# yekaizhou/duet

Measured on AMD Instinct MI355X. Metric: SV support-read marks clustered+phased /sec; bit-exact phased_sv.vcf vs ref, higher is better.
Workload: dtype u32/u64 integer + f64 threshold compares; 1 GPU; BASELINE configs[1]: synthetic 1 contig, 1001116 SV marks / 100000 candidates / 159991 tagged reads, resident in HBM; step = ef_classify + ef_finalize_own, two launches (phasing, E/F; ef_seed_sort 0: ; marks_per_gpu=1001116, candidates_per_gpu=100000, reads_per_gpu=159991, parallelism=contig-sharded x1, svlen_thres=50, suppread_thres=2, device_preheat_steps=2700

## Files before the change

### duet_amd/csrc/duet_ef.hip

```cpp

#include <hip/hip_runtime.h>
#include <hip/hip_ext.h>
#include <stdint.h>
#include <stdio.h>
#include <stdlib.h>
#include <string.h>
#include <string>
#include <vector>

#include "duet_ef.h"
#include "duet_internal.h"

#pragma clang fp contract(off)

namespace {

#ifdef DUET_STAMPS
#define STAMP(k, i) do { if (threadIdx.x == 0 && p.stamps) p.stamps[((size_t)(k) * 65536 + blockIdx.x) * 8 + (i)] = wall_clock64(); } while (0)
#else
#define STAMP(k, i) do { } while (0)
#endif

#include "duet_seeds.hip.h"

// ... 295 lines not shown
    const uint32_t s_a1 = a1 ? wave_sum(ta1) : 0u, s_a2 = a2 ? wave_sum(ta2) : 0u;
    const uint32_t s_b1 = b1 ? wave_sum(tb1) : 0u, s_b2 = b2 ? wave_sum(tb2) : 0u;
    if (lane == h) {
        st.first_ps = first_ps; st.multi = st.multi || multi;
        st.ps_a = ps_a; st.ps_b = ps_b; st.more = st.more || more;
        st.nv += nv; st.n_a += n_a; st.n_b += n_b;
        st.a1 += a1; st.a2 += a2; st.b1 += b1; st.b2 += b2;
        st.TA1 += s_a1; st.TA2 += s_a2; st.tb1 += s_b1; st.tb2 += s_b2;
    }
}

__device__ __forceinline__ void lds_barrier() { asm volatile("s_waitcnt lgkmcnt(0)\n\ts_barrier" ::: "memory"); }

struct TileRecs {
    const ulonglong4 *p;
    __device__ __forceinline__ ulonglong4 operator[](uint32_t b) const { return p[2 * (size_t)b]; }
    __device__ __forceinline__ ulonglong4 second(uint32_t b) const { return p[2 * (size_t)b + 1]; }
};

struct TileShared {
    uint32_t seed[kCandPerBlock];
    uint32_t wcnt[kCandPerBlock / 64], wlast[kCandPerBlock / 64], wclean[kCandPerBlock / 64];
    uint32_t c2n;
    uint32_t c2base;
};

__device__ __forceinline__ void store_summary(const Params &p, uint32_t slot, const CandState &st)
{
    uint32_t *rec = p.c2rec + (size_t)slot * kC2Words;
    const uint32_t ng = (st.n_a != 0) + (st.n_b != 0);
    rec[0] = st.nv; rec[1] = ng;
    rec[2] = st.ps_a; rec[3] = st.n_a; rec[4] = st.a1; rec[5] = st.a2;
    rec[6] = (uint32_t)st.TA1; rec[7] = (uint32_t)st.TA2;
    rec[8] = st.ps_b; rec[9] = st.n_b; rec[10] = st.b1; rec[11] = st.b2; rec[12] = st.tb1; rec[13] = st.tb2;
}

__device__ __forceinline__ uint32_t decide_store(const Params &p, TileShared &sh, uint32_t tile, bool live, uint32_t c,
                                                 bool active, bool divzero, const CandState &st, uint32_t deg,
                                                 uint32_t svread, uint32_t refread, uint32_t &c2_rank)
{
    uint8_t code = 0;
    uint32_t ps_out = 0;
    bool want_seed = false;
    const uint32_t n_ps = st.n_ps();
    const bool c2 = active && n_ps == 2;
    const bool c2_fast = c2 && !st.more && deg < 500000u;
    const uint32_t rank = c2_fast ? atomicAdd(&sh.c2n, 1u) : kEmpty;
    c2_rank = rank;
    if (live) {
        want_seed = (active || divzero) && (n_ps == 1) && st.seed() != kEmpty;
        if (divzero) {
            code = kDivZero;
        } else if (active) {
            if (c2) {
                if (rank < kC2Quota) {
                    const uint32_t slot = tile * kC2Quota + rank;
                    store_summary(p, slot, st);
                    code = kClass2;
                    ps_out = slot;
                } else {
                    code = kClass2Slow;
                }
            } else {
                Vote v;
                v.hap1 = st.a1; v.hap2 = st.a2; v.hap0 = 0;
                v.allhap = st.a1 + st.a2;
                v.t1 = st.TA1; v.t2 = st.TA2;
                bool need_fp = false;
                int pred = (p.dbg & DUET_DBG_EF_FP_DECIDE) ? 0 : decide01_int((int)n_ps, v, deg, svread, refread, need_fp);
                need_fp = need_fp || (p.dbg & DUET_DBG_EF_FP_DECIDE) != 0;
                if (need_fp) pred = decide((int)n_ps, v, deg, svread, refread);
                code = (uint8_t)pred;
                ps_out = st.ps_a == kEmpty ? 0u : st.ps_a;
                if (n_ps == 0 || (st.a1 == 0 && st.a2 == 0)) code |= kNeedNearest;
            }
        }
        p.out_pred[c] = code;
        p.out_ps[c] = ps_out;
    }
    return want_seed ? st.seed() : kEmpty;
}

__device__ __forceinline__ void seeds_tile(const Params &p, TileShared &sh, uint32_t tile, uint32_t tid, uint32_t c,
                                           uint32_t is_start)
{
    const uint32_t seed = sh.seed[tid];
    const bool want_seed = seed != kEmpty;
    const uint32_t lane = tid & 63u, wave = tid >> 6;
    const unsigned long long wmask = __ballot(want_seed);
    const unsigned long long smask = __ballot(is_start != 0);
    const unsigned long long upto = lane == 63 ? ~0ull : ((1ull << (lane + 1)) - 1ull);
    if (lane == 0) {
        if (wmask) {
            const uint32_t li = 63u - (uint32_t)__clzll(wmask);
            sh.wlast[wave] = sh.seed[wave * 64 + li];
            sh.wclean[wave] = (li == 63 || (smask >> (li + 1)) == 0) ? 1u : 0u;
        } else {
            sh.wlast[wave] = kEmpty;
            sh.wclean[wave] = 0;
        }
    }
    __syncthreads();
    bool keep = want_seed;
    if (want_seed) {
        const unsigned long long lower = wmask & (upto >> 1);
        if (lower) {
            const uint32_t pl = 63u - (uint32_t)__clzll(lower);
            const unsigned long long between = smask & upto & ~((1ull << (pl + 1)) - 1ull);
            keep = !(between == 0 && sh.seed[wave * 64 + pl] == seed);
        } else if (wave > 0) {
            keep = !((smask & upto) == 0 && sh.wclean[wave - 1] && sh.wlast[wave - 1] == seed);
        }
    }
    const unsigned long long mask = __ballot(keep);
    if (lane == 0) sh.wcnt[wave] = (uint32_t)__popcll(mask);
    __syncthreads();
    uint32_t before = 0, total = 0;
#pragma unroll
    for (uint32_t w = 0; w < kCandPerBlock / 64; ++w) {
        before += w < wave ? sh.wcnt[w] : 0u;
        total += sh.wcnt[w];
    }
    if (keep) {
        const uint32_t at = before + (uint32_t)__popcll(mask & (upto >> 1));
        const uint64_t e = ((uint64_t)c << 32) | seed;
        if (at < 7) p.blk_rec[(size_t)tile * 8 + 1 + at] = e;
        if (at >= 3) p.seed_ent[(size_t)tile * kCandPerBlock + at] = e;
    }
    if (tid == 0) p.blk_rec[(size_t)tile * 8] = total;
}

__device__ __forceinline__ void issue_fence()
{
    asm volatile("" ::: "memory");
    __builtin_amdgcn_sched_barrier(0);
}

__device__ __forceinline__ void stage_load_marks(const uint32_t *__restrict__ mark_read, uint4 (&r)[kStageIt], uint32_t cs, uint32_t m_end,
                                                 uint32_t tid)
{
#pragma unroll
    for (int it = 0; it < kStageIt; ++it) {
        const uint32_t m = cs + 4u * (tid + it * kCandPerBlock);
        r[it] = *reinterpret_cast<const uint4 *>(mark_read + (m < m_end ? m : cs));
    }
    issue_fence();
}

__device__ __forceinline__ void stage_gather(const uint64_t *__restrict__ read_tag, const uint64_t *__restrict__ untagged, uint32_t n_reads,
                                             uint64_t (&t)[4 * kStageIt], const uint4 (&r)[kStageIt])
{
#pragma unroll
    for (int it = 0; it < kStageIt; ++it) {
        uint32_t idx[4] = {r[it].x, r[it].y, r[it].z, r[it].w};
        asm volatile("" : "+v"(idx[0]), "+v"(idx[1]), "+v"(idx[2]), "+v"(idx[3])::"memory");
#pragma unroll
        for (int j = 0; j < 4; ++j) {
            const uint64_t *a = idx[j] < n_reads ? read_tag + idx[j] : untagged;
            t[4 * it + j] = *a;
        }
        issue_fence();
    }
}

__device__ __forceinline__ void stage_store(uint64_t *s_tag, const uint64_t (&t)[4 * kStageIt], uint32_t tid)
{
#pragma unroll
    for (int it = 0; it < kStageIt; ++it) {
        const uint32_t i = 4u * (tid + it * kCandPerBlock);
#pragma unroll
        for (int j = 0; j < 4; ++j) s_tag[i + j] = t[4 * it + j];
    }
}

template <bool VEC, bool DYN = false>
__global__ __launch_bounds__(kCandPerBlock, 6) void ef_classify(const Params p)
{
    __shared__ uint64_t s_tag[kChunk];
    __shared__ uint32_t s_span[2];
    __shared__ TileShared sh;

    const uint32_t tid = threadIdx.x;
    STAMP(0, 0);
    const uint32_t C = p.C, n_reads = p.n_reads, svlen_thres = p.svlen_thres, suppread_thres = p.suppread_thres;
    const uint32_t heavy_t = min(p.heavy_t, 255u);
    const uint32_t *__restrict__ const cand_off = p.cand_off, *__restrict__ const mark_read = p.mark_read;
    const uint64_t *__restrict__ const read_tag = p.read_tag, *__restrict__ const untagged = p.untagged;
    const uint32_t *__restrict__ const cand_svlen = p.cand_svlen, *__restrict__ const cand_svread = p.cand_svread;
    const uint32_t *__restrict__ const cand_refread = p.cand_refread;
    const uint8_t *__restrict__ const cand_gt_ok = p.cand_gt_ok, *__restrict__ const ctg_start = p.ctg_start;
    asm volatile("" ::"s"(C), "s"(n_reads), "s"(svlen_thres), "s"(suppread_thres), "s"(heavy_t), "s"(cand_off), "s"(mark_read),
                 "s"(read_tag), "s"(untagged), "s"(cand_svlen), "s"(cand_svread), "s"(cand_refread), "s"(cand_gt_ok), "s"(ctg_start));
    asm volatile("" ::"s"(p.dbg), "s"(p.out_pred), "s"(p.out_ps), "s"(p.blk_rec), "s"(p.seed_ent), "s"(p.c2rec), "s"(p.status),
                 "s"(p.c2_fixed), "s"(p.c2_cap));
    uint32_t n_cands = C;
    for (uint32_t tile = blockIdx.x;; tile += gridDim.x) {
        const uint32_t c0 = tile * kCandPerBlock, c = c0 + tid;
        const uint32_t ic = min(c, C - 1u);
        const uint32_t o0_ld = cand_off[min(c, C)], o1_ld = cand_off[min(c + 1u, C)];
        const uint32_t svlen_ld = cand_svlen[ic], svread_ld = cand_svread[ic], refread_ld = cand_refread[ic], gt_ld = cand_gt_ok[ic];
        uint32_t start_ld = 0, cc0_ld = 0, cc1_ld = 0, mb_ld = 0, me_ld = 0;
        if constexpr (DYN) {
            if (p.cand_contig) {
                cc0_ld = p.cand_contig[ic];
                cc1_ld = p.cand_contig[max(ic, 1u) - 1u];
            }
        } else {
            start_ld = ctg_start[ic];
            mb_ld = cand_off[c0];
            me_ld = cand_off[min(c0 + (uint32_t)kCandPerBlock, C)];
        }
        if constexpr (DYN) {
            uint32_t zero = 0;
            asm volatile("" : "+s"(zero));
            n_cands = p.dyn_c[zero];
            if (c0 >= n_cands) break;
        }
        const uint32_t nc = min((uint32_t)kCandPerBlock, n_cands - c0);
        asm volatile("" ::"v"(o0_ld), "v"(o1_ld), "v"(svlen_ld), "v"(svread_ld), "v"(refread_ld), "v"(gt_ld), "v"(start_ld), "v"(cc0_ld),
                     "v"(cc1_ld));
        if (tid == 0) sh.c2n = 0;
        const bool live = tid < nc;
        const uint32_t svlen = svlen_ld, svread = svread_ld, refread = refread_ld, gt_ok = gt_ld;
        uint32_t is_start = 0;
        if constexpr (DYN) {
            if (p.cand_contig) {
                is_start = (live && (c == 0 || cc0_ld != cc1_ld)) ? 1u : 0u;
            } else if (live) {
                uint32_t k = p.blk_ctg[tile];
                while (c >= p.ctg_off[k + 1]) ++k;
                is_start = c == p.ctg_off[k] ? 1u : 0u;
            }
        } else {
            is_start = live ? start_ld : 0u;
        }
        const bool kept = live && svlen >= svlen_thres && svread >= suppread_thres && gt_ok != 0;
        const bool divzero = kept && ((uint64_t)svread + (uint64_t)refread == 0);
        uint32_t m_begin, m_end;
        if constexpr (DYN) {
            if (tid == 0) s_span[0] = o0_ld;
            if (tid == nc - 1u) s_span[1] = o1_ld;
            lds_barrier();
            m_begin = s_span[0]; m_end = s_span[1];
        } else {
            m_begin = mb_ld; m_end = me_ld;
        }
        m_begin = (uint32_t)__builtin_amdgcn_readfirstlane((int)m_begin);
        m_end = (uint32_t)__builtin_amdgcn_readfirstlane((int)m_end);
        STAMP(0, 1);

        const uint32_t j = tid;
        const bool active = kept && !divzero;
        const uint32_t my_b = live ? o0_ld : 0, my_e = live ? o1_ld : 0;
        CandState st;

        const uint32_t base = VEC ? (m_begin & ~3u) : m_begin;
        for (uint32_t cs = base; cs < m_end; cs += kChunk) {
            if (VEC) {
                uint4 r[kStageIt];
                uint64_t t[4 * kStageIt];
                stage_load_marks(mark_read, r, cs, m_end, tid);
                stage_gather(read_tag, untagged, n_reads, t, r);
                stage_store(s_tag, t, tid);
            } else {
                for (uint32_t i = tid; i < kChunk && cs + i < m_end; i += kCandPerBlock) {
                    const uint32_t r = mark_read[cs + i];
                    s_tag[i] = r < n_reads ? read_tag[r] : kUntagged;
                }
            }
            __syncthreads();
            STAMP(0, 2);
            uint32_t lo = max(my_b, cs);
            const uint32_t hi = min(my_e, cs + (uint32_t)kChunk);
            if (!kept) lo = hi;
            const bool heavy = lo < hi && my_e - my_b > heavy_t;
            unsigned long long hm = __ballot(heavy);
            consume_range(st, s_tag, heavy ? hi : lo, hi, cs);
            while (hm) {
                const uint32_t h = (uint32_t)__builtin_amdgcn_readfirstlane((int)((uint32_t)__ffsll((long long)hm) - 1u));
                hm &= hm - 1ull;
                const uint32_t lo_h = (uint32_t)__builtin_amdgcn_readlane((int)lo, h), hi_h = (uint32_t)__builtin_amdgcn_readlane((int)hi, h);
                consume_heavy(st, s_tag, lo_h, hi_h, cs, tid & 63u, h);
            }
            STAMP(0, 3);
            __syncthreads();
        }
        STAMP(0, 4);
        uint32_t c2_rank;
        const uint32_t seed = decide_store(p, sh, tile, live, c0 + j, active, divzero, st, my_e - my_b, svread, refread, c2_rank);
        sh.seed[j] = seed;
        __syncthreads();
        if (sh.c2n > kC2Quota) {
            if (tid == 0) sh.c2base = atomicAdd(&p.status[1], sh.c2n - kC2Quota);
            __syncthreads();
            if (live && c2_rank != kEmpty && c2_rank >= kC2Quota) {
                const uint32_t at = sh.c2base + (c2_rank - kC2Quota);
                if (at < p.c2_cap - p.c2_fixed) {
                    store_summary(p, p.c2_fixed + at, st);
                    p.out_pred[c0 + j] = kClass2;
                    p.out_ps[c0 + j] = p.c2_fixed + at;
                }
            }
        }
        seeds_tile(p, sh, tile, tid, c0 + tid, is_start);
        STAMP(0, 6);
        if (!DYN) break;
        __syncthreads();
    }
}


__device__ void bitonic_sort(uint32_t *a, uint32_t n, uint32_t tid, uint32_t nthreads)
{
    uint32_t lN = 0;
    while ((1u << lN) < n) ++lN;
    const uint32_t pairs = (1u << lN) >> 1;
    for (uint32_t lk = 1; lk <= lN; ++lk) {
        const uint32_t k = 1u << lk, half = k >> 1;
        for (uint32_t i = tid; i < pairs; i += nthreads) {
            const uint32_t base = (i >> (lk - 1)) << lk, off = i & (half - 1);
            const uint32_t x = base + off, y = base + (k - 1 - off);
            if (y < n) {
                const uint32_t ax = a[x], ay = a[y];
                if (ax > ay) { a[x] = ay; a[y] = ax; }
            }
        }
        __syncthreads();
        for (int lj = (int)lk - 2; lj >= 0; --lj) {
            const uint32_t j = 1u << lj;
            for (uint32_t i = tid; i < pairs; i += nthreads) {
                const uint32_t x = ((i >> lj) << (lj + 1)) + (i & (j - 1)), y = x + j;
                if (y < n) {
                    const uint32_t ax = a[x], ay = a[y];
                    if (ax > ay) { a[x] = ay; a[y] = ax; }
                }
            }
            __syncthreads();
        }
    }
}

__device__ bool oddeven_rounds(uint32_t *a, uint32_t n, uint32_t tid, uint32_t nthreads, uint32_t *s_flag, int max_rounds)
{
    for (int r = 0; r < max_rounds; ++r) {
        if (tid == 0) *s_flag = 0;
        __syncthreads();
        for (int par = 0; par < 2; ++par) {
            for (uint32_t i = 2 * tid + par; i + 1 < n; i += 2 * nthreads) {
                const uint32_t x = a[i], y = a[i + 1];
                if (x > y) { a[i] = y; a[i + 1] = x; *s_flag = 1; }
            }
            __syncthreads();
        }
        if (*s_flag == 0) return true;
        __syncthreads();
    }
    return false;
}

__device__ uint32_t block_exscan(uint32_t v, uint32_t tid, uint32_t *s_part , uint32_t nthreads,
                                 uint32_t *total)
{
    const uint32_t lane = tid & 63u, wave = tid >> 6;
    uint32_t x = v;
#pragma unroll
    for (int d = 1; d < 64; d <<= 1) {
        const uint32_t y = __shfl_up(x, d, 64);
        if ((int)lane >= d) x += y;
    }
    if (lane == 63) s_part[wave] = x;
    __syncthreads();
    uint32_t before = 0, tot = 0;
    for (uint32_t w = 0; w < nthreads / 64; ++w) {
        const uint32_t pw = s_part[w];
        before += w < wave ? pw : 0u;
        tot += pw;
    }
    __syncthreads();
    *total = tot;
    return before + x - v;
}

__device__ uint32_t unique_copy(const uint32_t *src, uint32_t n, uint32_t *dst, uint32_t tid, uint32_t nthreads,
                                uint32_t *s_part)
{
    const uint32_t per = (n + nthreads - 1) / nthreads;
    const uint32_t b = min(n, tid * per), e = min(n, b + per);
    uint32_t cnt = 0;
    for (uint32_t i = b; i < e; ++i) cnt += (i == 0 || src[i] != src[i - 1]);
    uint32_t total;
    uint32_t at = block_exscan(cnt, tid, s_part, nthreads, &total);
// ... 1349 lines not shown
    if (ctx->cl_fork) (void)hipEventDestroy(ctx->cl_fork);
    if (ctx->sv_depth_off_ev) (void)hipEventDestroy(ctx->sv_depth_off_ev);
    if (ctx->plan_ev) (void)hipEventDestroy(ctx->plan_ev);
    if (ctx->plan_stage) (void)hipHostFree(ctx->plan_stage);
    delete ctx;
}

int duet_ctx_set_profiling(duet_ctx *ctx, int enabled)
{
    if (!ctx) return fail(nullptr, DUET_ERR_INVALID, "null context");
    if (ctx->ev_used && ctx->ev_mode != (enabled == 3 ? 1 : enabled))
        return fail(ctx, DUET_ERR_INVALID, "collect the pending profile before changing the mode");
    ctx->profiling = enabled < 0 ? 0 : (enabled > 3 ? 3 : enabled);
    ctx->prof_tick = 0;
    return DUET_OK;
}

#ifdef DUET_STAMPS
DUET_API int duet_dbg_stamps(duet_ctx *ctx, int enable, unsigned long long *host_out)
{
    const size_t bytes = (size_t)6 * 65536 * 8 * 8;
    if (enable && !ctx->d_stamps) { if (hipMalloc((void **)&ctx->d_stamps, bytes) != hipSuccess) return -1; }
    if (enable) { (void)hipMemset(ctx->d_stamps, 0, bytes); return 0; }
    if (ctx->d_stamps && host_out) { (void)hipDeviceSynchronize(); (void)hipMemcpy(host_out, ctx->d_stamps, bytes, hipMemcpyDeviceToHost); }
    return 0;
}
#endif

int duet_ctx_set_debug(duet_ctx *ctx, uint32_t flags)
{
    if (!ctx) return fail(nullptr, DUET_ERR_INVALID, "null context");
    ctx->dbg = flags;
    return DUET_OK;
}

int duet_ef_run_device(duet_ctx *ctx, const duet_ef_problem *pr, uint8_t *out_pred, uint32_t *out_ps, void *stream_)
{
    int rc = validate(ctx, pr, out_pred, out_ps);
    if (rc) return rc;
    hipStream_t stream = (hipStream_t)stream_;
    HIP_TRY(ctx, hipSetDevice(ctx->device));
    if (pr->n_cands == 0) return DUET_OK;
    if ((rc = ensure_plan(ctx, pr, stream))) return rc;

    Params p;
    memset(&p, 0, sizeof(p));
    p.K = pr->n_contigs; p.C = pr->n_cands; p.M = pr->n_marks;
    p.read_tag = pr->n_reads ? pr->read_tag : (const uint64_t *)ctx->d_n_one;
    p.n_reads = pr->n_reads; p.untagged = ctx->d_untagged;
    p.cand_pos = pr->cand_pos; p.cand_svlen = pr->cand_svlen; p.cand_svread = pr->cand_svread;
    p.cand_refread = pr->cand_refread; p.cand_gt_ok = pr->cand_gt_ok;
    p.cand_off = pr->cand_off; p.mark_read = pr->mark_read;
    p.svlen_thres = pr->svlen_thres; p.suppread_thres = pr->suppread_thres;
    p.ctg_off = ctx->d_ctg_off; p.ctg_start = (const uint8_t *)ctx->ws_start.ptr; p.blk_ctg = ctx->d_blk_ctg;
    p.blk_rec = (uint64_t *)ctx->d_blk_cnt; p.seed_ent = (uint64_t *)ctx->ws_ent.ptr;
    p.one_cap = pr->n_cands + pr->n_contigs;
    p.n_small = pr->n_contigs <= (uint32_t)kSmallK ? pr->n_contigs : 0;
    for (uint32_t k = 0; k <= p.n_small && p.n_small; ++k) p.ctg_small[k] = pr->cand_ctg_off[k];
    p.onebuf = (uint32_t *)ctx->ws_one.ptr; p.tmpbuf = (uint32_t *)ctx->ws_tmp.ptr;
    p.n_one = ctx->d_n_one; p.c2rec = (uint32_t *)ctx->ws_c2.ptr; p.status = ctx->d_status;
    p.c2_fixed = ((p.C + kCandPerBlock - 1) / kCandPerBlock) * kC2Quota;
    p.c2_cap = (uint32_t)c2_slots((p.C + kCandPerBlock - 1) / kCandPerBlock, p.C);
    p.out_pred = out_pred; p.out_ps = out_ps;
    p.dbg = ctx->dbg;
    p.heavy_t = (ctx->dbg & DUET_DBG_EF_HEAVY_ALL) ? 0u : ((ctx->dbg & DUET_DBG_EF_HEAVY_OFF) ? 0xFFFFFFFFu : ctx->ef_heavy_t);
    p.stamps = ctx->d_stamps;

    hipEvent_t ev[6] = {nullptr, nullptr, nullptr, nullptr, nullptr, nullptr};
    int prof = ctx->profiling;
    if (prof == 3) prof = (ctx->prof_tick++ % 8u == 0) ? 1 : 0;
    if (prof) {
        ctx->ev_mode = prof;
        while (ctx->ev_pool.size() < ctx->ev_used + 6) {
            hipEvent_t e;
            HIP_TRY(ctx, hipEventCreate(&e));
            ctx->ev_pool.push_back(e);
        }
        for (int i = 0; i < (prof == 2 ? 6 : 2); ++i) ev[i] = ctx->ev_pool[ctx->ev_used + i];
        ctx->ev_used += 6;
    }
    const uint32_t blocks = (pr->n_cands + kCandPerBlock - 1) / kCandPerBlock;
    const uint32_t three = DUET_DBG_EF_OWN_OFF | DUET_DBG_EF_FIN_TPB2 | DUET_DBG_EF_FIN_TPB4 | DUET_DBG_EF_NO_SEED_HASH;
    const bool own = p.n_small && !(ctx->dbg & three) && (blocks <= kOwnMaxTiles || (ctx->dbg & DUET_DBG_EF_OWN_ALL));
    if (prof) ctx->ev_kmask.push_back(own ? 0x5 : 0x7);
    if (((uintptr_t)pr->mark_read & 15) == 0)
        hipExtLaunchKernelGGL(ef_classify<true>, dim3(blocks), dim3(kCandPerBlock), 0, stream, ev[0], ev[1], 0, p);
    else
        hipExtLaunchKernelGGL(ef_classify<false>, dim3(blocks), dim3(kCandPerBlock), 0, stream, ev[0], ev[1], 0, p);
    if (own) {
        hipExtLaunchKernelGGL(ef_finalize_own, dim3(blocks), dim3(256), 0, stream, ev[4], ev[5], 0, p);
        ctx->ef_last_params.assign((const unsigned char *)&p, (const unsigned char *)&p + sizeof(p));
        ctx->ef_last_stream = stream;
        ctx->ef_seeds_stale = true;
    } else {
        ctx->ef_seeds_stale = false;
        hipExtLaunchKernelGGL(ef_seed_sort, dim3(pr->n_contigs), dim3(kSortThreads), 0, stream, ev[2], ev[3], 0, p);
        const uint32_t C = pr->n_cands;
        int tpb = (!p.n_small || C < 1000000u) ? 1 : (C < 8000000u ? 2 : 4);
        if (p.n_small && (ctx->dbg & DUET_DBG_EF_FIN_TPB2)) tpb = 2;
        if (p.n_small && (ctx->dbg & DUET_DBG_EF_FIN_TPB4)) tpb = 4;
        if (tpb == 4) hipExtLaunchKernelGGL((ef_finalize<false, 4>), dim3((C + 1023) / 1024), dim3(256), 0, stream, ev[4], ev[5], 0, p);
        else if (tpb == 2) hipExtLaunchKernelGGL((ef_finalize<false, 2>), dim3((C + 511) / 512), dim3(256), 0, stream, ev[4], ev[5], 0, p);
        else hipExtLaunchKernelGGL((ef_finalize<false, 1>), dim3((C + 255) / 256), dim3(256), 0, stream, ev[4], ev[5], 0, p);
    }
    HIP_TRY(ctx, hipGetLastError());
    ctx->pending_check = true;
    return DUET_OK;
}

}

int duet_ef_plan_on_device_prepare(duet_ctx *ctx, uint32_t K, uint32_t c_max, hipStream_t stream, uint32_t **ctg_off_out,
                                   uint32_t **zero_out)
{
    const uint32_t C = c_max;
    const uint32_t B = (C + kCandPerBlock - 1) / kCandPerBlock;
    const size_t small_words = (size_t)(K + 1) + K + 8 + (size_t)B + 16 + (size_t)B * 16;
    const size_t want[6] = {small_words * 4, C, (size_t)B * kCandPerBlock * 8, ((size_t)C + K + 1) * 4, ((size_t)C + K + 1) * 4,
                            c2_slots(B, C) * kC2Words * 4};
    DevBuf *bufs[6] = {&ctx->ws_small, &ctx->ws_start, &ctx->ws_ent, &ctx->ws_one, &ctx->ws_tmp, &ctx->ws_c2};
    bool grow = ctx->plan_stream != stream;
    for (int i = 0; i < 6; ++i) grow = grow || want[i] > bufs[i]->cap;
    int rc;
    if (grow) {
        HIP_TRY(ctx, hipDeviceSynchronize());
        for (int i = 0; i < 6; ++i)
            if ((rc = reserve(ctx, *bufs[i], want[i]))) return rc;
    }
    uint32_t *w = (uint32_t *)ctx->ws_small.ptr;
    ctx->d_ctg_off = w;            w += K + 1;
    ctx->d_n_one = w;              w += K;
    ctx->d_status = w;             w += 8;
    ctx->d_blk_ctg = w;            w += B;
    w += ((uintptr_t)w & 63) ? (64 - ((uintptr_t)w & 63)) / 4 : 0;
    ctx->d_blk_cnt = w;
    ctx->plan_off.clear();
    ctx->plan_C = 0;
    ctx->plan_stream = stream;
    if (ctg_off_out) *ctg_off_out = ctx->d_ctg_off;
    if (zero_out) *zero_out = ctx->d_n_one;
    return DUET_OK;
}

int duet_ef_run_planned_on_device(duet_ctx *ctx, const duet_ef_problem *pr, uint32_t c_max, const uint32_t *d_n_cands,
                                  const uint32_t *d_ctg_off, const uint16_t *d_cand_contig, uint8_t *out_pred, uint32_t *out_ps,
                                  hipStream_t stream, bool planned)
{
    const uint32_t K = pr->n_contigs, C = c_max;
    if (K == 0 || C == 0) return DUET_OK;
    const uint32_t B = (C + kCandPerBlock - 1) / kCandPerBlock;
    int rc;
    if ((rc = duet_ef_plan_on_device_prepare(ctx, K, c_max, stream, nullptr, nullptr))) return rc;
    if (!planned) {
        const uint32_t nthr = B > K + 8 ? B : K + 8;
        if (d_cand_contig)
            hipLaunchKernelGGL(plan_device_contigs, dim3((nthr + 255) / 256), dim3(256), 0, stream, d_cand_contig, d_n_cands, K, B,
                               ctx->d_ctg_off, ctx->d_n_one, ctx->d_blk_ctg);
        else
            hipLaunchKernelGGL(plan_device, dim3((nthr + 255) / 256), dim3(256), 0, stream, d_ctg_off, K, B, ctx->d_ctg_off,
                               ctx->d_n_one, ctx->d_blk_ctg);
    }

    Params p;
    memset(&p, 0, sizeof(p));
    p.K = K; p.C = C; p.M = pr->n_marks;
    p.dyn_c = d_n_cands;
    p.cand_contig = d_cand_contig;
    p.read_tag = pr->n_reads ? pr->read_tag : (const uint64_t *)ctx->d_n_one;
// ... 179 lines not shown
```

### include/duet_ef.h

```cpp
#ifndef DUET_EF_H
#define DUET_EF_H

#include <stdint.h>

#ifdef __cplusplus
extern "C" {
#endif

#define DUET_ABI_VERSION 1

#define DUET_API __attribute__((visibility("default")))

typedef enum duet_status {
    DUET_OK = 0,
    DUET_ERR_INVALID = -1,
    DUET_ERR_NO_DEVICE = -2,
    DUET_ERR_HIP = -3,
    DUET_ERR_OOM = -4,
    DUET_ERR_TIMEOUT = -6,
    DUET_ERR_DIV_ZERO = -5
} duet_status;

#define DUET_TAG(hap, pc, ps) (((uint64_t)(hap) << 62) | ((uint64_t)(pc) << 32) | (uint64_t)(uint32_t)(ps))
#define DUET_MARK_ABSENT 0xFFFFFFFFu
#define DUET_PC_MAX 8100u

typedef struct duet_ef_problem {
    uint32_t n_contigs;
    uint32_t n_cands;
    uint32_t n_marks;
    uint32_t n_reads;
    const uint32_t *cand_ctg_off;
    const uint64_t *read_tag;
    const uint32_t *cand_pos;
    const uint32_t *cand_svlen;
    const uint32_t *cand_svread;
    const uint32_t *cand_refread;
    const uint8_t *cand_gt_ok;
    const uint32_t *cand_off;
    const uint32_t *mark_read;
    uint32_t svlen_thres;
    uint32_t suppread_thres;
} duet_ef_problem;

enum { DUET_K_CLASSIFY = 0, DUET_K_SEEDS = 1, DUET_K_FINALIZE = 2, DUET_N_KERNELS = 3 };

typedef struct duet_ef_stats {
    uint64_t algorithmic_bytes;
    uint32_t n_seed_ps;
    uint32_t n_profiled_runs;
    float kernel_ms[DUET_N_KERNELS];
    float total_ms;
} duet_ef_stats;

typedef struct duet_ctx duet_ctx;

DUET_API int duet_abi_version(void);

DUET_API duet_ctx *duet_ctx_create(int device_id);
DUET_API void duet_ctx_destroy(duet_ctx *ctx);
DUET_API const char *duet_last_error(const duet_ctx *ctx);

DUET_API int duet_ctx_set_profiling(duet_ctx *ctx, int mode);

DUET_API int duet_ef_run_device(duet_ctx *ctx, const duet_ef_problem *prob, uint8_t *out_pred, uint32_t *out_ps,
                       void *stream);

DUET_API int duet_ef_check(duet_ctx *ctx, void *stream);

DUET_API int duet_ef_run_host(duet_ctx *ctx, const duet_ef_problem *prob, uint8_t *out_pred, uint32_t *out_ps,
                     duet_ef_stats *stats);

DUET_API int duet_ef_profile_collect(duet_ctx *ctx, duet_ef_stats *stats);

#define DUET_DBG_EF_NO_SEED_HASH 0x40u
#define DUET_DBG_EF_FIN_TPB2 0x20u
#define DUET_DBG_EF_FIN_TPB4 0x80u
#define DUET_DBG_EF_HEAVY_ALL 0x80000u
#define DUET_DBG_EF_HEAVY_OFF 0x100000u
#define DUET_DBG_EF_FP_DECIDE 0x400000u
#define DUET_DBG_EF_OWN_OFF 0x800000u
#define DUET_DBG_EF_OWN_ALL 0x1000000u
#define DUET_DBG_EF_OWN_SMALLTAB 0x2000000u
#define DUET_DBG_CLUSTER_EVENT_FORKS 0x4000000u
#define DUET_DBG_CLUSTER_WIDE_OFF 0x8000000u
#define DUET_DBG_CLUSTER_EXACT 0x100u
#define DUET_DBG_CLUSTER_LARGE 0x200u
#define DUET_DBG_CLUSTER_PAIRS 0x400u
#define DUET_DBG_CLUSTER_NOBOX 0x800u
#define DUET_DBG_CLUSTER_KEYSORT 0x10000u
#define DUET_DBG_CLUSTER_RECSORT 0x40000u
#define DUET_DBG_CLUSTER_NOSYM 0x20000u
#define DUET_DBG_CLUSTER_LSD 0x8000u
#define DUET_DBG_CLUSTER_SMALLCAP 0x4000u
#define DUET_DBG_CLUSTER_TIERS 0x2000u
#define DUET_DBG_CLUSTER_KC2 0x1000u
DUET_API int duet_ctx_set_debug(duet_ctx *ctx, uint32_t flags);

DUET_API int duet_ef_get_seed_ps(duet_ctx *ctx, uint32_t contig, uint32_t *out, uint32_t cap);

typedef struct duet_cluster_problem {
    uint32_t n_marks;
    uint32_t part_gap;
    uint32_t part_max;
    uint32_t n_contigs_hint;
    uint32_t n_types_hint;
    uint32_t max_pos_hint;
    uint32_t max_span_hint;
    uint32_t reserved;
    double max_dist;
    double normalizer;
    const uint16_t *mark_contig;
    const uint8_t *mark_type;
    const uint32_t *mark_pos;
    const uint32_t *mark_span;
} duet_cluster_problem;

typedef struct duet_cluster_result {
    uint32_t *order;
    uint32_t *cand_off;
    uint16_t *cand_contig;
    uint8_t *cand_type;
    uint32_t *cand_pos;
    uint32_t *cand_span;
    uint32_t *n_cands;
} duet_cluster_result;

DUET_API int duet_cluster_run_device(duet_ctx *ctx, const duet_cluster_problem *prob, const duet_cluster_result *res,
                            void *stream);
DUET_API int duet_cluster_run_host(duet_ctx *ctx, const duet_cluster_problem *prob, const duet_cluster_result *res);

typedef struct duet_svim_problem {
    duet_cluster_problem marks;
    const uint32_t *mark_read;
    const uint64_t *read_tag;
    uint32_t n_reads;
    uint32_t n_contigs;
    const uint32_t *depth;
    const uint32_t *depth_off;
    uint32_t depth_bin;
    uint32_t svlen_thres, suppread_thres;
    uint32_t reserved;
} duet_svim_problem;

DUET_API int duet_svim_phase_device(duet_ctx *ctx, const duet_svim_problem *prob, const duet_cluster_result *res,
                           uint8_t *out_pred, uint32_t *out_ps, uint32_t *n_cands_host, void *stream);

DUET_API int duet_svim_phase_host(duet_ctx *ctx, const duet_svim_problem *prob, const duet_cluster_result *res,
                         uint8_t *out_pred, uint32_t *out_ps);

typedef struct duet_callset_names {
    const uint32_t *mark_name;
    const uint64_t *name_off;
    const char *name_pool;
    uint32_t n_names;
    uint32_t n_contigs;
    const char *const *chrom;
} duet_callset_names;

DUET_API int duet_svim_vcf_rows_device(duet_ctx *ctx, const duet_svim_problem *prob, const duet_cluster_result *res, uint32_t n_cands,
                                       const duet_callset_names *names, char *out_text, uint64_t out_cap, uint64_t *out_len,
                                       void *stream);
// ... 299 lines not shown
```

Measured before the change: 61.99 billion marks/s.

## Split each candidate's mark range across two threads in a wider classify kernel

```diff
diff --git a/duet_amd/csrc/duet_ef.hip b/duet_amd/csrc/duet_ef.hip
--- a/duet_amd/csrc/duet_ef.hip
+++ b/duet_amd/csrc/duet_ef.hip
@@ -401,15 +401,15 @@
 }
 
 __device__ __forceinline__ void seeds_tile(const Params &p, TileShared &sh, uint32_t tile, uint32_t tid, uint32_t c,
-                                           uint32_t is_start)
-{
-    const uint32_t seed = sh.seed[tid];
+                                           uint32_t is_start, bool owner = true)
+{
+    const uint32_t seed = owner ? sh.seed[tid] : kEmpty;
     const bool want_seed = seed != kEmpty;
     const uint32_t lane = tid & 63u, wave = tid >> 6;
     const unsigned long long wmask = __ballot(want_seed);
     const unsigned long long smask = __ballot(is_start != 0);
     const unsigned long long upto = lane == 63 ? ~0ull : ((1ull << (lane + 1)) - 1ull);
-    if (lane == 0) {
+    if (lane == 0 && owner) {
         if (wmask) {
             const uint32_t li = 63u - (uint32_t)__clzll(wmask);
             sh.wlast[wave] = sh.seed[wave * 64 + li];
@@ -432,7 +432,7 @@
         }
     }
     const unsigned long long mask = __ballot(keep);
-    if (lane == 0) sh.wcnt[wave] = (uint32_t)__popcll(mask);
+    if (lane == 0 && owner) sh.wcnt[wave] = (uint32_t)__popcll(mask);
     __syncthreads();
     uint32_t before = 0, total = 0;
 #pragma unroll
@@ -455,22 +455,24 @@
     __builtin_amdgcn_sched_barrier(0);
 }
 
-__device__ __forceinline__ void stage_load_marks(const uint32_t *__restrict__ mark_read, uint4 (&r)[kStageIt], uint32_t cs, uint32_t m_end,
+template <int NT = kCandPerBlock, int IT>
+__device__ __forceinline__ void stage_load_marks(const uint32_t *__restrict__ mark_read, uint4 (&r)[IT], uint32_t cs, uint32_t m_end,
                                                  uint32_t tid)
 {
 #pragma unroll
-    for (int it = 0; it < kStageIt; ++it) {
-        const uint32_t m = cs + 4u * (tid + it * kCandPerBlock);
+    for (int it = 0; it < IT; ++it) {
+        const uint32_t m = cs + 4u * (tid + it * NT);
         r[it] = *reinterpret_cast<const uint4 *>(mark_read + (m < m_end ? m : cs));
     }
     issue_fence();
 }
 
+template <int IT>
 __device__ __forceinline__ void stage_gather(const uint64_t *__restrict__ read_tag, const uint64_t *__restrict__ untagged, uint32_t n_reads,
-                                             uint64_t (&t)[4 * kStageIt], const uint4 (&r)[kStageIt])
-{
-#pragma unroll
-    for (int it = 0; it < kStageIt; ++it) {
+                                             uint64_t (&t)[4 * IT], const uint4 (&r)[IT])
+{
+#pragma unroll
+    for (int it = 0; it < IT; ++it) {
         uint32_t idx[4] = {r[it].x, r[it].y, r[it].z, r[it].w};
         asm volatile("" : "+v"(idx[0]), "+v"(idx[1]), "+v"(idx[2]), "+v"(idx[3])::"memory");
 #pragma unroll
@@ -482,11 +484,12 @@
     }
 }
 
-__device__ __forceinline__ void stage_store(uint64_t *s_tag, const uint64_t (&t)[4 * kStageIt], uint32_t tid)
-{
-#pragma unroll
-    for (int it = 0; it < kStageIt; ++it) {
-        const uint32_t i = 4u * (tid + it * kCandPerBlock);
+template <int NT = kCandPerBlock, int IT4>
+__device__ __forceinline__ void stage_store(uint64_t *s_tag, const uint64_t (&t)[IT4], uint32_t tid)
+{
+#pragma unroll
+    for (int it = 0; it < IT4 / 4; ++it) {
+        const uint32_t i = 4u * (tid + it * NT);
 #pragma unroll
         for (int j = 0; j < 4; ++j) s_tag[i + j] = t[4 * it + j];
     }
@@ -626,6 +629,173 @@
         if (!DYN) break;
         __syncthreads();
     }
+}
+
+constexpr int kSplit = 2;
+constexpr int kSplitThreads = kSplit * kCandPerBlock;
+constexpr int kSplitChunk = kChunk;
+constexpr int kSplitStagers = 384;
+constexpr int kSplitStageIt = kSplitChunk / (kSplitStagers * 4);
+constexpr uint32_t kSplitMaxTiles = 512;
+static_assert(kSplit == 2 || kSplit == 4, "the parts are halves, or halves of halves");
+static_assert(kSplitStageIt >= 1 && kSplitStageIt * kSplitStagers * 4 == kSplitChunk, "a pass is whole 16-byte loads");
+static_assert(kSplitStagers % 64 == 0 && kSplitStagers <= kSplitThreads, "whole wavefronts stage");
+
+__device__ __forceinline__ void split_bounds(uint32_t b, uint32_t e, uint32_t part, uint32_t &lo, uint32_t &hi)
+{
+    lo = b; hi = e;
+#pragma unroll
+    for (uint32_t bit = kSplit >> 1; bit != 0; bit >>= 1) {
+        const uint32_t mid = lo + (hi - lo + 1u) / 2u;
+        if (part & bit) lo = mid; else hi = mid;
+    }
+}
+
+__device__ __forceinline__ void fold(CandState &l, const CandState &r)
+{
+    l.multi = l.multi || r.multi || (l.first_ps != kEmpty && r.first_ps != kEmpty && l.first_ps != r.first_ps);
+    l.first_ps = min(l.first_ps, r.first_ps);
+    l.nv += r.nv;
+    auto take = [&](uint32_t ps, uint32_t n, uint32_t h1, uint32_t h2, uint32_t t1, uint32_t t2) {
+        const bool is = ps != kEmpty;
+        const bool to_a = is && (l.ps_a == kEmpty || l.ps_a == ps);
+        const bool to_b = is && !to_a && (l.ps_b == kEmpty || l.ps_b == ps);
+        l.ps_a = to_a ? ps : l.ps_a;
+        l.a1 += to_a ? h1 : 0u; l.a2 += to_a ? h2 : 0u;
+        l.TA1 += to_a ? t1 : 0u; l.TA2 += to_a ? t2 : 0u;
+        l.ps_b = to_b ? ps : l.ps_b;
+        l.n_b += to_b ? n : 0u;
+        l.b1 += to_b ? h1 : 0u; l.b2 += to_b ? h2 : 0u;
+        l.tb1 += to_b ? t1 : 0u; l.tb2 += to_b ? t2 : 0u;
+        l.more = l.more || (is && !to_a && !to_b);
+    };
+    take(r.ps_a, r.nv - r.n_b, r.a1, r.a2, (uint32_t)r.TA1, (uint32_t)r.TA2);
+    take(r.ps_b, r.n_b, r.b1, r.b2, r.tb1, r.tb2);
+    l.more = l.more || r.more;
+    l.n_a = l.more ? (l.ps_a != kEmpty ? 1u : 0u) : l.nv - l.n_b;
+}
+
+__device__ __forceinline__ void hand_store(uint4 (*s_hand)[(kSplit - 1) * kCandPerBlock], uint32_t slot, const CandState &st)
+{
+    s_hand[0][slot] = make_uint4(st.first_ps, st.ps_a, st.ps_b, st.nv | st.n_b << 8 | (st.multi ? 1u << 16 : 0u) | (st.more ? 1u << 17 : 0u));
+    s_hand[1][slot] = make_uint4(st.a1 << 24 | (uint32_t)st.TA1, st.a2 << 24 | (uint32_t)st.TA2, st.b1 << 24 | st.tb1, st.b2 << 24 | st.tb2);
+}
+
+__device__ __forceinline__ CandState hand_load(const uint4 (*s_hand)[(kSplit - 1) * kCandPerBlock], uint32_t slot)
+{
+    const uint4 x = s_hand[0][slot], y = s_hand[1][slot];
+    CandState st;
+    st.first_ps = x.x; st.ps_a = x.y; st.ps_b = x.z;
+    st.nv = x.w & 0xFFu; st.n_b = (x.w >> 8) & 0xFFu; st.multi = (x.w >> 16 & 1u) != 0; st.more = (x.w >> 17 & 1u) != 0;
+    st.a1 = y.x >> 24; st.a2 = y.y >> 24; st.b1 = y.z >> 24; st.b2 = y.w >> 24;
+    st.TA1 = y.x & 0xFFFFFFu; st.TA2 = y.y & 0xFFFFFFu; st.tb1 = y.z & 0xFFFFFFu; st.tb2 = y.w & 0xFFFFFFu;
+    return st;
+}
+
+template <bool VEC>
+__global__ __launch_bounds__(kSplitThreads, 6) void ef_classify_split(const Params p)
+{
+    __shared__ uint64_t s_tag[kSplitChunk];
+    __shared__ uint4 s_hand[2][(kSplit - 1) * kCandPerBlock];
+    __shared__ TileShared sh;
+
+    const uint32_t tid = threadIdx.x, j = tid % kCandPerBlock, part = tid / kCandPerBlock;
+    const bool owner = part == 0;
+    STAMP(0, 0);
+    const uint32_t C = p.C, n_reads = p.n_reads, svlen_thres = p.svlen_thres, suppread_thres = p.suppread_thres;
+    const uint32_t heavy_t = min(p.heavy_t, 255u);
+    const uint32_t *__restrict__ const cand_off = p.cand_off, *__restrict__ const mark_read = p.mark_read;
+    const uint64_t *__restrict__ const read_tag = p.read_tag, *__restrict__ const untagged = p.untagged;
+    const uint32_t *__restrict__ const cand_svlen = p.cand_svlen, *__restrict__ const cand_svread = p.cand_svread;
+    const uint32_t *__restrict__ const cand_refread = p.cand_refread;
+    const uint8_t *__restrict__ const cand_gt_ok = p.cand_gt_ok, *__restrict__ const ctg_start = p.ctg_start;
+    asm volatile("" ::"s"(C), "s"(n_reads), "s"(svlen_thres), "s"(suppread_thres), "s"(heavy_t), "s"(cand_off), "s"(mark_read),
+                 "s"(read_tag), "s"(untagged), "s"(cand_svlen), "s"(cand_svread), "s"(cand_refread), "s"(cand_gt_ok), "s"(ctg_start));
+    asm volatile("" ::"s"(p.dbg), "s"(p.out_pred), "s"(p.out_ps), "s"(p.blk_rec), "s"(p.seed_ent), "s"(p.c2rec), "s"(p.status),
+                 "s"(p.c2_fixed), "s"(p.c2_cap));
+    const uint32_t tile = blockIdx.x, c0 = tile * kCandPerBlock, c = c0 + j;
+    const uint32_t ic = min(c, C - 1u);
+    const uint32_t o0_ld = cand_off[min(c, C)], o1_ld = cand_off[min(c + 1u, C)];
+    const uint32_t svlen_ld = cand_svlen[ic], svread_ld = cand_svread[ic], refread_ld = cand_refread[ic], gt_ld = cand_gt_ok[ic];
+    const uint32_t start_ld = ctg_start[ic];
+    const uint32_t mb_ld = cand_off[c0], me_ld = cand_off[min(c0 + (uint32_t)kCandPerBlock, C)];
+    const uint32_t nc = min((uint32_t)kCandPerBlock, C - c0);
+    asm volatile("" ::"v"(o0_ld), "v"(o1_ld), "v"(svlen_ld), "v"(svread_ld), "v"(refread_ld), "v"(gt_ld), "v"(start_ld));
+    if (tid == 0) sh.c2n = 0;
+    const bool live = j < nc;
+    const uint32_t svlen = svlen_ld, svread = svread_ld, refread = refread_ld, gt_ok = gt_ld;
+    const uint32_t is_start = (owner && live) ? start_ld : 0u;
+    const bool kept = live && svlen >= svlen_thres && svread >= suppread_thres && gt_ok != 0;
+    const bool divzero = kept && ((uint64_t)svread + (uint64_t)refread == 0);
+    const uint32_t m_begin = (uint32_t)__builtin_amdgcn_readfirstlane((int)mb_ld);
+    const uint32_t m_end = (uint32_t)__builtin_amdgcn_readfirstlane((int)me_ld);
+    STAMP(0, 1);
+
+    const bool active = kept && !divzero;
+    const uint32_t my_b = live ? o0_ld : 0, my_e = live ? o1_ld : 0;
+    const bool heavy_c = my_e - my_b > heavy_t;
+    uint32_t w_b, w_e;
+    split_bounds(my_b, my_e, part, w_b, w_e);
+    if (heavy_c) { w_b = my_b; w_e = owner ? my_e : my_b; }
+    if (!kept) w_e = w_b;
+    CandState st;
+
+    const uint32_t base = VEC ? (m_begin & ~3u) : m_begin;
+    for (uint32_t cs = base; cs < m_end; cs += kSplitChunk) {
+        if (VEC) {
+            if (tid < kSplitStagers) {
+                uint4 r[kSplitStageIt];
+                uint64_t t[4 * kSplitStageIt];
+                stage_load_marks<kSplitStagers>(mark_read, r, cs, m_end, tid);
+                stage_gather(read_tag, untagged, n_reads, t, r);
+                stage_store<kSplitStagers>(s_tag, t, tid);
+            }
+        } else {
+            for (uint32_t i = tid; i < kSplitChunk && cs + i < m_end; i += kSplitThreads) {
+                const uint32_t r = mark_read[cs + i];
+                s_tag[i] = r < n_reads ? read_tag[r] : kUntagged;
+            }
+        }
+        __syncthreads();
+        STAMP(0, 2);
+        const uint32_t lo = max(w_b, cs), hi = min(w_e, cs + (uint32_t)kSplitChunk);
+        const bool heavy = heavy_c && lo < hi;
+        unsigned long long hm = __ballot(heavy);
+        consume_range(st, s_tag, heavy ? hi : lo, hi, cs);
+        while (hm) {
+            const uint32_t h = (uint32_t)__builtin_amdgcn_readfirstlane((int)((uint32_t)__ffsll((long long)hm) - 1u));
+            hm &= hm - 1ull;
+            const uint32_t lo_h = (uint32_t)__builtin_amdgcn_readlane((int)lo, h), hi_h = (uint32_t)__builtin_amdgcn_readlane((int)hi, h);
+            consume_heavy(st, s_tag, lo_h, hi_h, cs, tid & 63u, h);
+        }
+        STAMP(0, 3);
+        if (!owner && cs + (uint32_t)kSplitChunk >= m_end) hand_store(s_hand, tid - kCandPerBlock, st);
+        __syncthreads();
+    }
+    STAMP(0, 4);
+    uint32_t c2_rank = kEmpty;
+    if (owner) {
+        if (base < m_end) {
+#pragma unroll
+            for (int k = 1; k < kSplit; ++k) fold(st, hand_load(s_hand, (k - 1) * kCandPerBlock + j));
+        }
+        sh.seed[j] = decide_store(p, sh, tile, live, c, active, divzero, st, my_e - my_b, svread, refread, c2_rank);
+    }
+    __syncthreads();
+    if (sh.c2n > kC2Quota) {
+        if (tid == 0) sh.c2base = atomicAdd(&p.status[1], sh.c2n - kC2Quota);
+        __syncthreads();
+        if (owner && live && c2_rank != kEmpty && c2_rank >= kC2Quota) {
+            const uint32_t at = sh.c2base + (c2_rank - kC2Quota);
+            if (at < p.c2_cap - p.c2_fixed) {
+                store_summary(p, p.c2_fixed + at, st);
+                p.out_pred[c] = kClass2;
+                p.out_ps[c] = p.c2_fixed + at;
+            }
+        }
+    }
+    seeds_tile(p, sh, tile, tid, c, is_start, owner);
+    STAMP(0, 6);
 }
 
 
@@ -2141,8 +2311,13 @@
     const uint32_t blocks = (pr->n_cands + kCandPerBlock - 1) / kCandPerBlock;
     const uint32_t three = DUET_DBG_EF_OWN_OFF | DUET_DBG_EF_FIN_TPB2 | DUET_DBG_EF_FIN_TPB4 | DUET_DBG_EF_NO_SEED_HASH;
     const bool own = p.n_small && !(ctx->dbg & three) && (blocks <= kOwnMaxTiles || (ctx->dbg & DUET_DBG_EF_OWN_ALL));
+    const bool split = own && blocks <= kSplitMaxTiles && !(ctx->dbg & DUET_DBG_EF_SPLIT_OFF);
     if (prof) ctx->ev_kmask.push_back(own ? 0x5 : 0x7);
-    if (((uintptr_t)pr->mark_read & 15) == 0)
+    if (split && ((uintptr_t)pr->mark_read & 15) == 0)
+        hipExtLaunchKernelGGL(ef_classify_split<true>, dim3(blocks), dim3(kSplitThreads), 0, stream, ev[0], ev[1], 0, p);
+    else if (split)
+        hipExtLaunchKernelGGL(ef_classify_split<false>, dim3(blocks), dim3(kSplitThreads), 0, stream, ev[0], ev[1], 0, p);
+    else if (((uintptr_t)pr->mark_read & 15) == 0)
         hipExtLaunchKernelGGL(ef_classify<true>, dim3(blocks), dim3(kCandPerBlock), 0, stream, ev[0], ev[1], 0, p);
     else
         hipExtLaunchKernelGGL(ef_classify<false>, dim3(blocks), dim3(kCandPerBlock), 0, stream, ev[0], ev[1], 0, p);
diff --git a/include/duet_ef.h b/include/duet_ef.h
--- a/include/duet_ef.h
+++ b/include/duet_ef.h
@@ -78,6 +78,7 @@
 #define DUET_DBG_EF_FIN_TPB4 0x80u
 #define DUET_DBG_EF_HEAVY_ALL 0x80000u
 #define DUET_DBG_EF_HEAVY_OFF 0x100000u
+#define DUET_DBG_EF_SPLIT_OFF 0x200000u
 #define DUET_DBG_EF_FP_DECIDE 0x400000u
 #define DUET_DBG_EF_OWN_OFF 0x800000u
 #define DUET_DBG_EF_OWN_ALL 0x1000000u
```

Measured after the change: 63.25 billion marks/s (median of 6 runs). +2.0%, better.
